# sandialabs/tenzing

Hardware: AMD Instinct MI355X
Metric: best-schedule iter time (ms) + MCTS search wall-clock, 3D halo-exchange 8 ranks (lower is better)
Workload: dtype fp64

## Files before the change

### tenzing_amd/csrc/bind/module.cpp

```cpp
#include <pybind11/functional.h>
#include <pybind11/pybind11.h>
#include <pybind11/stl.h>

#include "core/benchmark.hpp"
#include "core/health.hpp"
#include "core/solve.hpp"
#include "hip/comm_ops.hpp"
#include "hip/hip_runtime.hpp"
#include "hip/rccl_comm.hpp"
#include "hip/rocsparse_spmv.hpp"
#include "kernels/kernels.hpp"
#include "workloads/workloads.hpp"

#include <hip/hip_runtime_api.h>

#include <csignal>
#include <cstdlib>
#include <execinfo.h>
#include <sstream>
#include <unistd.h>
#include <vector>

namespace py = pybind11;
using namespace tz;
// ... 930 lines not shown
      .def_readwrite("hostsplit_fracs", &HaloArgs::hostsplit_fracs)
      .def_readwrite("hostsplit_chunks", &HaloArgs::hostsplit_chunks)
      .def_readwrite("wide_puts", &HaloArgs::wide_puts)
      .def_readwrite("wide_put_blocks", &HaloArgs::wide_put_blocks)
      .def_readwrite("ipc_grid", &HaloArgs::ipc_grid)
      .def_readwrite("copy_puts", &HaloArgs::copy_puts)
      .def_readwrite("copy_engines", &HaloArgs::copy_engines)
      .def_readwrite("move_pairs", &HaloArgs::move_pairs)
      .def_readwrite("grid_memory", &HaloArgs::grid_memory)
      .def_readwrite("node_tag", &HaloArgs::node_tag)
      .def_readwrite("device", &HaloArgs::device)
      .def("json", [](const HaloArgs &a) { return a.json().dump(); });
  py::class_<HaloExchange, std::shared_ptr<HaloExchange>>(m, "HaloExchange")
      .def(py::init([](const HaloArgs &a) { return std::make_shared<HaloExchange>(a); }))
      .def_property_readonly("args", &HaloExchange::args)
      .def("ndirs", &HaloExchange::ndirs)
      .def("dir_name", [](const HaloExchange &h, int i) { return h.dir(i).name(); })
      .def("dir", [](const HaloExchange &h, int i) { auto d = h.dir(i); return py::make_tuple(d.dx, d.dy, d.dz); })
      .def("opposite", &HaloExchange::opposite)
      .def("neighbor", &HaloExchange::neighbor)
      .def("coords", &HaloExchange::coords)
      .def("rank_grid", &HaloExchange::rank_grid)
      .def("box_elems", &HaloExchange::box_elems)
      .def("pack_box", [](const HaloExchange &h, int i) { return box_to_dict(h.pack_box(i)); })
      .def("unpack_box", [](const HaloExchange &h, int i) { return box_to_dict(h.unpack_box(i)); })
      .def_static("chunk_box",
                  [](const py::dict &b, int parts) {
                    py::list out;
                    for (const kern::BoxDesc &c : HaloExchange::chunk_box(box_from_dict(b), parts))
                      out.append(box_to_dict(c));
                    return out;
                  },
                  py::arg("box"), py::arg("parts"))
      .def("grid_elems", &HaloExchange::grid_elems)
      .def("grid_memory", &HaloExchange::grid_memory, "fine or coarse (HaloArgs.grid_memory)")
      .def("off_node_dirs", &HaloExchange::off_node_dirs,
           "remote directions whose neighbour runs on another node (RCCL only)")
      .def("layout", [](const HaloExchange &h) {
             const kern::HaloGeom g = h.geom();
             py::dict d;
             d["order"] = g.order == 0 ? "xyzq" : "qxyz";
             d["x_offset_cells"] = g.xoff;
             d["row_pitch_elems"] = g.sy;
             d["grid_bytes"] = double(h.grid_elems()) * 8.0;
             const bool q = g.order == 1;
             d["strides_qzyx"] = py::make_tuple(q ? 1 : g.sq, g.sz, g.sy, q ? int64_t(g.nq) : 1);
             d["shape_qzyx"] = py::make_tuple(g.nq, g.nz + 2 * g.g, g.ny + 2 * g.g, g.nx + 2 * g.g);
             d["ghost"] = g.g;
             return d;
           }, "storage layout: order, x padding before the first ghost cell, row pitch")
      .def("exchange_bytes", &HaloExchange::exchange_bytes)
      .def("setup", [](HaloExchange &h, Ctrl *c) { h.setup(c); }, py::arg("ctrl") = nullptr,
           py::call_guard<py::gil_scoped_release>())
      .def("ready", &HaloExchange::ready)
      .def("add_to_graph", &HaloExchange::add_to_graph)
      .def("grid_ptr", [](const HaloExchange &h) { return reinterpret_cast<uintptr_t>(h.grid()); })
      .def("read_grid", [](HaloExchange &h, uintptr_t dst, uintptr_t s) { h.copy_grid(P(dst), false, P(s)); },
           py::arg("dst"), py::arg("stream") = 0, "copy grid_elems() doubles of storage to dst")
      .def("write_grid", [](HaloExchange &h, uintptr_t src, uintptr_t s) { h.copy_grid(P(src), true, P(s)); },
           py::arg("src"), py::arg("stream") = 0, "overwrite the grid storage from src")
      .def("init_grid", [](HaloExchange &h, uintptr_t s, int gen) { h.init_grid(P(s), gen); },
           py::arg("stream") = 0, py::arg("gen") = 0)
      .def("check_grid", [](HaloExchange &h, uintptr_t s) { return h.check_grid(P(s)); }, py::arg("stream") = 0)
      .def("check_stencil", [](HaloExchange &h, uintptr_t s) { return h.check_stencil(P(s)); }, py::arg("stream") = 0)
      .def("stencil", [](const HaloExchange &h, int region, uintptr_t s) { h.stencil(region, P(s)); },
           py::arg("region"), py::arg("stream") = 0)
// ... 312 lines not shown
```

### tenzing_amd/csrc/workloads/halo.cpp

```cpp
#include "halo_internal.hpp"

#include <functional>
#include <map>

#include "core/health.hpp"
#include "core/solve.hpp"

#include <algorithm>
#include <chrono>
#include <thread>

namespace tz {

Json HaloArgs::json() const {
  Json j;
  j["nx"] = nx;
  j["ny"] = ny;
  j["nz"] = nz;
  j["nq"] = nq;
  j["ghost"] = ghost;
  j["neighbors"] = neighbors;
  j["order"] = order;
  j["transport"] = transport;
  j["fuse"] = fuse;
// ... 148 lines not shown
  copyEngines_ = a_.copy_engines;

  TZ_CHECK(a_.relay == "auto" || a_.relay == "off" || a_.relay == "force",
           "relay must be auto, off or force (got " << a_.relay << ")");
  TZ_CHECK(!a_.relay_fracs.empty(), "relay_fracs is empty");
  for (double f : a_.relay_fracs) TZ_CHECK(f > 0.0 && f < 0.5, "relay fraction " << f << " not in (0, 0.5)");
  bool facesIpc = true;
  for (int i : group_dirs(1)) facesIpc = facesIpc && ipc_[i];
  relay_ = a_.relay != "off" && a_.px == 2 && a_.py == 2 && a_.pz == 2 && useIpc_ && !ipcGrid_ && facesIpc;
  TZ_CHECK(a_.relay != "force" || relay_,
           "relay routing forced but needs a 2x2x2 rank grid with ipc puts in buffers mode");
  TZ_CHECK(a_.hostsplit == "auto" || a_.hostsplit == "off" || a_.hostsplit == "force",
           "hostsplit must be auto, off or force (got " << a_.hostsplit << ")");
  TZ_CHECK(!a_.hostsplit_fracs.empty(), "hostsplit_fracs is empty");
  for (double f : a_.hostsplit_fracs)
    TZ_CHECK(f > 0.0 && f < 1.0, "host share " << f << " not in (0, 1)");
  TZ_CHECK(a_.hostsplit_chunks >= 1 && a_.hostsplit_chunks <= 8,
           "hostsplit_chunks must be 1..8 (got " << a_.hostsplit_chunks << ")");
  hsChunks_ = a_.hostsplit_chunks;
  bool anyFace = false;
  for (int i : group_dirs(1)) anyFace = anyFace || ipc_[i];
  hsOffered_ = a_.hostsplit != "off" && useIpc_ && !ipcGrid_ && anyFace;
  TZ_CHECK(a_.hostsplit != "force" || hsOffered_,
           "host split forced but needs remote faces with ipc puts in buffers mode");
  corner_ = coord_to_rank(cx_ + 1, cy_ + 1, cz_ + 1);
  relayOrigin_ = coord_to_rank(cx_ - 1, cy_ - 1, cz_ - 1);
  fwdTo_.assign(dirs_.size(), -1);
  fwdFrom_.assign(dirs_.size(), -1);
  for (size_t i = 0; i < dirs_.size(); ++i) {
    const Dir &d = dirs_[i];
    fwdTo_[i] = coord_to_rank(cx_ - 1 + d.dx, cy_ - 1 + d.dy, cz_ - 1 + d.dz);
    fwdFrom_[i] = coord_to_rank(cx_ - d.dx + 1, cy_ - d.dy + 1, cz_ - d.dz + 1);
  }
}

HaloExchange::~HaloExchange() {
  if (recoveryHook_) remove_recovery_hook(recoveryHook_);
  for (auto &kv : engines_) {
    for (void *e : kv.second.events) (void)hipEventDestroy(static_cast<hipEvent_t>(e));
    for (void *s : kv.second.streams) (void)hipStreamDestroy(static_cast<hipStream_t>(s));
  }
  for (void *p : opened_) (void)hipIpcCloseMemHandle(p);
  if (flags_) (void)hipFree(flags_);
}

int HaloExchange::coord_to_rank(int x, int y, int z) const {
  auto w = [](int v, int n) { return ((v % n) + n) % n; };
  return w(x, a_.px) + a_.px * (w(y, a_.py) + a_.py * w(z, a_.pz));
}

static void axis_range(int d, int n, int g, bool ghost, int &lo, int &ext) {
  if (d == 0) {
    lo = g;
    ext = n;
  } else if (d < 0) {
    lo = ghost ? 0 : g;
    ext = g;
  } else {
    lo = ghost ? n + g : n;
    ext = g;
  }
}

kern::BoxDesc halo_detail::make_box(const HaloArgs &a, const HaloExchange::Dir &d, bool ghost,
                                    int64_t xoff, int64_t sy, int64_t sz, int64_t sq) {
  int x0, ex, y0, ey, z0, ez;
  axis_range(d.dx, a.nx, a.ghost, ghost, x0, ex);
  axis_range(d.dy, a.ny, a.ghost, ghost, y0, ey);
  axis_range(d.dz, a.nz, a.ghost, ghost, z0, ez);
  kern::BoxDesc b;
  if (a.order == "xyzq") {
    b.grid_off = z0 * sz + y0 * sy + x0 + xoff;
    b.len = ex;
    b.n1 = ey;
    b.n2 = ez;
    b.n3 = a.nq;
    b.s1 = sy;
    b.s2 = sz;
    b.s3 = sq;
  } else {
    b.grid_off = int64_t(a.nq) * (x0 + xoff) + y0 * sy + z0 * sz;
    b.len = a.nq * ex;
    b.n1 = ey;
    b.n2 = ez;
    b.n3 = 1;
    b.s1 = sy;
    b.s2 = sz;
    b.s3 = 0;
  }
  return b;
}

kern::BoxDesc HaloExchange::pack_box(int i) const {
  kern::BoxDesc b = make_box(a_, dirs_[i], false, xoff_, sy_, sz_, sq_);
  if (!send_.empty()) b.buf = send_[i].as<double>();
  return b;
}

kern::BoxDesc HaloExchange::unpack_box(int i) const {
  kern::BoxDesc b = make_box(a_, dirs_[i], true, xoff_, sy_, sz_, sq_);
  if (!recv_.empty()) b.buf = recv_[i].as<double>();
  ghost_widening(dirs_[i].dx, b.grid_off, b.len, b.lead, b.trail);
  return b;
}

size_t HaloExchange::box_elems(int i) const {
  kern::BoxDesc b = make_box(a_, dirs_[i], false, xoff_, sy_, sz_, sq_);
  return size_t(b.len) * b.n1 * b.n2 * b.n3;
}

double HaloExchange::exchange_bytes() const {
  double s = 0;
  for (int i = 0; i < ndirs(); ++i) s += 8.0 * double(box_elems(i));
  return s;
}

kern::HaloGeom HaloExchange::geom() const {
  kern::HaloGeom g;
  g.order = a_.order == "xyzq" ? 0 : 1;
  g.xoff = xoff_;
  g.sy = sy_;
  g.sz = sz_;
  g.sq = sq_;
  g.nx = a_.nx;
  g.ny = a_.ny;
  g.nz = a_.nz;
  g.nq = a_.nq;
  g.g = a_.ghost;
  g.cx = cx_;
  g.cy = cy_;
  g.cz = cz_;
  g.px = a_.px;
  g.py = a_.py;
  g.pz = a_.pz;
// ... 6 lines not shown
  if (ready()) return;
  ctrl_ = ctrl;
  if (a_.device >= 0) TZ_HIP(hipSetDevice(a_.device));
  TZ_CHECK(a_.grid_memory >= -1 && a_.grid_memory <= 1, "grid_memory must be -1 (auto), 0 or 1");
  if (useIpc_ && ctrl && ctrl->size() > 1) {
    const std::vector<std::string> ids = ctrl->allgather(node_identity() + a_.node_tag);
    TZ_CHECK(int(ids.size()) == a_.size, "allgather returned " << ids.size() << " entries");
    std::vector<double> off(size_t(ndirs()), 0.0);
    for (int i = 0; i < ndirs(); ++i)
      if (ipc_[i] && ids[size_t(nbr_[i])] != ids[size_t(a_.rank)]) off[size_t(i)] = 1.0;
    ctrl->allreduce_max(off.data(), int(off.size()));
    offNode_.assign(size_t(ndirs()), 0);
    int n = 0;
    for (int i = 0; i < ndirs(); ++i)
      if (off[size_t(i)] != 0.0) {
        offNode_[size_t(i)] = 1;
        ipc_[i] = false;
        ++n;
      }
    if (n > 0) {
      TZ_CHECK(a_.transport == "auto", "transport " << a_.transport << ": " << n
                   << " directions have a neighbour on another node, which IPC cannot reach "
                      "(transport auto sends them over RCCL)");
      useIpc_ = std::any_of(ipc_.begin(), ipc_.end(), [](bool b) { return b; });
      relay_ = false;
      hsOffered_ = false;
      useCopy_ = useIpc_ && a_.copy_puts;
      TZ_LOG(Info, "halo: " << n << " directions cross nodes (RCCL), "
                            << std::count(ipc_.begin(), ipc_.end(), true) << " stay on IPC");
    }
  }
  gridFine_ = a_.grid_memory < 0 ? useIpc_ && ipcGrid_ : a_.grid_memory != 0;
  grid_ = DeviceBuffer(gridElems_ * sizeof(double), gridFine_);
  send_.resize(ndirs());
  recv_.resize(ndirs());
  for (int i = 0; i < ndirs(); ++i) {
    if (direct_[i]) continue;
    if (pipe_[i] || (ipc_[i] && useCopy_ && !ipcGrid_)) send_[i] = DeviceBuffer(box_elems(i) * sizeof(double));
    if (pipe_[i] || (ipc_[i] && !ipcGrid_))
      recv_[i] = DeviceBuffer((box_elems(opp_[i]) + 16 * ((relay_ ? 1 : 0) + (hsOffered_ ? hsChunks_ + 1 : 0))) *
                                  sizeof(double),
                              ipc_[i] && !ipcGrid_);
  }
  if (relay_) {
    relayBuf_.resize(ndirs());
    for (int i : relay_faces()) {
      size_t most = 0;
      for (double f : a_.relay_fracs) {
        kern::BoxDesc A, B;
        split_box(make_box(a_, dirs_[i], false, xoff_, sy_, sz_, sq_), f, A, B);
        most = std::max(most, size_t(B.len) * B.n1 * B.n2 * B.n3);
      }
      relayBuf_[i] = DeviceBuffer(most * sizeof(double), true);
    }
  }
  const std::string failEnv = std::getenv("TZ_FAIL_TRANSPORTS") ? std::getenv("TZ_FAIL_TRANSPORTS") : "";
  auto simulated = [&](const std::string &what) {
    return ("," + failEnv + ",").find("," + what + ",") != std::string::npos;
  };
  if (useIpc_) {
    std::string why = setup_ipc(ctrl);
    if (why.empty() && simulated("ipc")) why = "simulated failure (TZ_FAIL_TRANSPORTS)";
    double failed = why.empty() ? 0.0 : 1.0;
    ctrl->allreduce_max(&failed, 1);
    ipcReady_ = failed == 0.0;
    if (!ipcReady_) {
      ipcWhy_ = why.empty() ? "failed on another rank" : why;
      TZ_LOG(Warn, "ipc transport unavailable: " << ipcWhy_);
      TZ_CHECK(a_.transport != "ipc", "ipc transport requested but unavailable: " << why);
    }
    if (relay_) {
      double bad = relayWhy_.empty() ? 0.0 : 1.0;
      ctrl->allreduce_max(&bad, 1);
      relayReady_ = ipcReady_ && bad == 0.0;
      if (ipcReady_ && !relayReady_) {
        TZ_LOG(Warn, "relay routing unavailable"
// ... 36 lines not shown
    ctrl->allreduce_max(&failed, 1);
    if (failed != 0.0) drop_rccl(why.empty() ? "communicator creation failed on another rank" : why);
  }
  init_grid();
  if (useRccl_) {
    const std::string why = rccl_preflight(*ctrl);
    if (!why.empty()) {
      drop_rccl("preflight: " + why);
    } else {
      if (!rcclGraphOk_) TZ_LOG(Warn, "RCCL ops run eagerly only: " << rcclGraphWhy_);
      TZ_LOG(Info, "rccl preflight passed (" << comms_.size() << " communicators of "
                                             << rccl_nranks() << " ranks)"
                                             << (rcclGraphOk_ ? ", " + rcclCaptureNote_ : ", eager only"));
    }
    init_grid();
  }
  if (useIpc_ && ipcReady_) {
    TZ_HIP(hipDeviceSynchronize());
    ctrl->barrier();
    ipc_preflight(ctrl);
    if (ipcReady_ && useCopy_ && !ipcGrid_) copy_preflight(ctrl);
    if (ipcReady_) wide_put_preflight(ctrl);
    if (relay_ && ipcReady_) relay_preflight(ctrl);
    if (hsReady_ && ipcReady_) hostsplit_preflight(ctrl);
  }
  bool piped = false;
  for (int i = 0; i < ndirs(); ++i) piped = piped || pipe_[i];
  if (piped && !useRccl_ && a_.transport != "copy" && !useHost_) {
    if (!off_node_dirs().empty() && useIpc_ && ipcReady_) {
      ipcReady_ = false;
      ipcWhy_ = "RCCL unavailable for the directions that cross nodes: host-staged transport";
    }
    if (useIpc_ && ipcReady_) {
      for (int i = 0; i < ndirs(); ++i) {
        if (pipe_[i]) {
          pipe_[i] = false;
          if (!(ipc_[i] && useCopy_ && !ipcGrid_)) send_[i] = DeviceBuffer();
          if (ipcGrid_) recv_[i] = DeviceBuffer();
        }
      }
    } else {
      TZ_CHECK(a_.transport == "auto", "RCCL transport unavailable and no fallback: " << rcclWhy_);
      useHost_ = true;
      TZ_LOG(Warn, "no device transport works (rccl: " << rcclWhy_ << "; ipc: "
                                                     << (useIpc_ ? ipcWhy_ : "not offered")
                                                     << "): the host-staged transport carries "
                                                        "the remote directions");
    }
  }
  TZ_HIP(hipDeviceSynchronize());
  if (useIpc_ && ipcReady_) {
    ctrl->barrier();
    recoveryHook_ = add_recovery_hook([this](Ctrl &c) { reset_ipc_counters(&c); });
  }
}

void HaloExchange::drop_rccl(const std::string &why) {
  for (auto &c : comms_)
    if (c && !c->aborted()) c->abort();
  comms_.clear();
  useRccl_ = false;
  rcclWhy_ = why;
  TZ_LOG(Warn, "RCCL transport unavailable: " << why);
}

int HaloExchange::rccl_nranks() const { return comms_.empty() ? 0 : comms_.front()->size(); }

std::map<std::string, std::string> HaloExchange::transport_report() const {
  std::map<std::string, std::string> r;
  const bool remote = std::any_of(nbr_.begin(), nbr_.end(), [&](int n) { return n != a_.rank; });
  const std::string &t = a_.transport;
  if (useRccl_)
    r["rccl"] = rcclGraphOk_ ? (rcclCaptureNote_.empty() ? "ok" : "ok (hipGraph: " + rcclCaptureNote_ + ")")
// ... 225 lines not shown
  TZ_HIP(hipStreamSynchronize(s));
}

void HaloExchange::check_pipelined(int i) const {
  TZ_CHECK(i >= 0 && i < ndirs(), "direction " << i << " out of range");
  TZ_CHECK(!direct_[i], "direction " << dirs_[i].name()
                                     << " uses the direct transport (no pack/transfer/unpack)");
  TZ_CHECK(pipe_[i] || ipc_[i], "direction " << dirs_[i].name() << " has no staging buffers");
  TZ_CHECK(ready(), "halo not set up");
}

void HaloExchange::pack(int i, void *stream) const {
  check_pipelined(i);
  kern::box_copy(grid(), pack_box(i), false, stream);
}

void HaloExchange::unpack(int i, void *stream) const {
  check_pipelined(i);
  kern::box_copy(grid(), unpack_box(i), true, stream);
}

const RcclComm &HaloExchange::comm_for(int streamIdx, int dir) const {
  TZ_CHECK(!comms_.empty(), "no RCCL communicators");
  const int k = streamIdx >= 0 ? streamIdx : dir;
  return *comms_[size_t(k) % comms_.size()];
}

void HaloExchange::shift(int i, void *stream, int streamIdx) const {
  check_pipelined(i);
  const int o = opp_[i];
  const size_t n = box_elems(i);
  if (useRccl_) {
    const RcclComm &c = comm_for(streamIdx, i);
    c.sendrecv(send_[i].get(), n, nbr_[i], recv_[o].get(), n, nbr_[o], 1, stream);
  } else {
    TZ_CHECK(nbr_[i] == a_.rank, "shift " << dirs_[i].name() << ": the neighbour is remote and RCCL "
                                          "is not in use (host transport: he_hostxfer)");
    kern::CopyDesc c{recv_[o].get(), send_[i].get(), n * sizeof(double)};
    kern::copy_many(&c, 1, stream);
  }
}

std::vector<int> HaloExchange::all_dirs() const {
  std::vector<int> v;
  for (int i = 0; i < ndirs(); ++i) v.push_back(i);
  return v;
}

std::vector<int> HaloExchange::group_dirs(int k) const {
  std::vector<int> v;
  for (int i = 0; i < ndirs(); ++i) {
    const int a = (dirs_[i].dx != 0) + (dirs_[i].dy != 0) + (dirs_[i].dz != 0);
    if (a == k || (k == 0 && a >= 2)) v.push_back(i);
  }
  return v;
}

void HaloExchange::pack_group(const std::vector<int> &dirs, void *stream) const {
  std::vector<kern::BoxDesc> bs;
  for (int i : dirs) {
    check_pipelined(i);
    bs.push_back(pack_box(i));
  }
  for (size_t k = 0; k < bs.size(); k += kern::kMaxBoxes)
    kern::box_copy_many(grid(), bs.data() + k, int(std::min<size_t>(kern::kMaxBoxes, bs.size() - k)),
                        false, stream);
}

void HaloExchange::unpack_group(const std::vector<int> &dirs, void *stream) const {
  std::vector<kern::BoxDesc> bs;
  for (int i : dirs) {
    check_pipelined(i);
    bs.push_back(unpack_box(opp_[i]));
  }
  for (size_t k = 0; k < bs.size(); k += kern::kMaxBoxes)
    kern::box_copy_many(grid(), bs.data() + k, int(std::min<size_t>(kern::kMaxBoxes, bs.size() - k)),
                        true, stream);
}

void HaloExchange::shift_group(const std::vector<int> &dirs, void *stream, int streamIdx) const {
  if (dirs.empty()) return;
  for (int i : dirs) check_pipelined(i);
  if (useRccl_) {
    std::vector<RcclComm::Xfer> xs;
    for (int i : dirs) {
      const int o = opp_[i];
      const size_t n = box_elems(i);
      xs.push_back({send_[i].get(), n, nbr_[i], recv_[o].get(), n, nbr_[o]});
    }
    comm_for(streamIdx, dirs.front()).exchange(xs, 1, stream);
  } else {
    std::vector<kern::CopyDesc> cs;
    for (int i : dirs) {
      TZ_CHECK(nbr_[i] == a_.rank, "shift " << dirs_[i].name() << ": the neighbour is remote and "
                                            "RCCL is not in use (host transport: he_hostxfer)");
      cs.push_back({recv_[opp_[i]].get(), send_[i].get(), box_elems(i) * sizeof(double)});
    }
    for (size_t k = 0; k < cs.size(); k += kern::kMaxBoxes)
      kern::copy_many(cs.data() + k, int(std::min<size_t>(kern::kMaxBoxes, cs.size() - k)), stream);
  }
}

std::vector<kern::MoveDesc> HaloExchange::direct_moves(const std::vector<int> &dirs_in) const {
  std::vector<int> dirs = dirs_in;
  std::stable_sort(dirs.begin(), dirs.end(), [&](int a, int b) {
    auto k = [&](int i) { return (dirs_[i].dx != 0) + (dirs_[i].dy != 0) + (dirs_[i].dz != 0); };
    return k(a) < k(b);
  });
  std::vector<kern::MoveDesc> ms;
  for (int i : dirs) {
    TZ_CHECK(i >= 0 && i < ndirs() && direct_[i], "direction " << i << " is not a direct (self) transfer");
    const kern::BoxDesc s = make_box(a_, dirs_[i], false, xoff_, sy_, sz_, sq_);
    const kern::BoxDesc d = make_box(a_, dirs_[opp_[i]], true, xoff_, sy_, sz_, sq_);
    kern::MoveDesc m;
    m.src = grid();
    m.dst = grid();
    m.src_off = s.grid_off;
    m.dst_off = d.grid_off;
    m.s1 = s.s1;
    m.s2 = s.s2;
    m.s3 = s.s3;
    m.len = s.len;
    m.n1 = s.n1;
    m.n2 = s.n2;
    m.n3 = s.n3;
    if (a_.ghost_align > 0) widen_to_sectors(dirs_[opp_[i]].dx, m);
    ms.push_back(m);
  }
  if (a_.order == "xyzq" && a_.move_pairs) ms = pair_x_moves(ms);
// ... 144 lines not shown
  } else {
    const int64_t end = dstOff % rowLen + len;
    const int64_t e = (A - (dstOff + len) % A) % A;
    if (end + e <= rowLen) trail = int32_t(e);
  }
}

void HaloExchange::widen_to_sectors(int ghostDx, kern::MoveDesc &m) const {
  int32_t lead = 0, trail = 0;
  ghost_widening(ghostDx, m.dst_off, m.len, lead, trail);
  m.src_off -= lead;
  m.dst_off -= lead;
  m.len += lead + trail;
}

std::vector<int> HaloExchange::pipelined_dirs() const {
  std::vector<int> v;
  for (int i = 0; i < ndirs(); ++i)
    if (!direct_[i]) v.push_back(i);
  return v;
}

void HaloExchange::host_exchange(const std::vector<int> &dirs_in) const {
  TZ_CHECK(ready() && ctrl_, "halo not set up");
  std::vector<int> dirs = dirs_in;
  std::sort(dirs.begin(), dirs.end());
  std::vector<std::string> out(size_t(a_.size));
  for (int i : dirs) {
    check_pipelined(i);
    const size_t bytes = box_elems(i) * sizeof(double);
    std::string &o = out[size_t(nbr_[i])];
    const size_t at = o.size();
    o.resize(at + bytes);
    TZ_HIP(hipMemcpy(&o[at], send_[i].get(), bytes, hipMemcpyDeviceToHost));
  }
  const std::vector<std::string> in = ctrl_->alltoallv(out);
  std::vector<size_t> used(in.size(), 0);
  for (int i : dirs) {
    const int o = opp_[i];
    const size_t from = size_t(nbr_[o]);
    const size_t bytes = box_elems(i) * sizeof(double);
    TZ_CHECK(from < in.size() && used[from] + bytes <= in[from].size(),
             "host exchange: rank " << from << " sent " << in[from].size() << " bytes, fewer than expected");
    TZ_HIP(hipMemcpy(recv_[o].get(), in[from].data() + used[from], bytes, hipMemcpyHostToDevice));
    used[from] += bytes;
  }
  for (size_t r = 0; r < in.size(); ++r)
    TZ_CHECK(used[r] == in[r].size(), "host exchange: rank " << r << " sent " << in[r].size()
                                                              << " bytes, expected " << used[r]);
}

void HaloExchange::pack_all(void *stream) const { pack_group(pipelined_dirs(), stream); }
void HaloExchange::unpack_all(void *stream) const { unpack_group(pipelined_dirs(), stream); }
void HaloExchange::shift_all(void *stream) const { shift_group(pipelined_dirs(), stream); }

}
```

### tenzing_amd/csrc/workloads/halo_ipc.cpp

```cpp
#include "halo_internal.hpp"

namespace tz {

void HaloExchange::off_node_exchange(void *stream) const {
  const std::vector<int> far = off_node_dirs();
  if (far.empty()) return;
  TZ_CHECK(useRccl_, "directions that cross nodes need the RCCL transport");
  for (int i : far) pack(i, stream);
  for (int i : far) shift(i, stream);
  for (int i : far) unpack(opp_[i], stream);
}

void HaloExchange::ipc_preflight(Ctrl *ctrl) {
  std::vector<int> local, remote;
  for (int i = 0; i < ndirs(); ++i) {
    if (direct_[i]) local.push_back(i);
    else if (ipc_[i]) remote.push_back(i);
  }
  double bad = 0;
  std::string why;
  const double keep = ipcTimeoutS_;
  ipcTimeoutS_ = std::min(ipcTimeoutS_, preflight_wait_s());
  for (int gen = 1; gen <= 2 && bad == 0; ++gen) {
    if (gen > 1) {
// ... 174 lines not shown
  init_grid();
}

std::string HaloExchange::setup_ipc(Ctrl *ctrl) {
  TZ_CHECK(ctrl && ctrl->size() == a_.size, "ipc transport needs a control plane of size " << a_.size);
  if (const char *v = std::getenv("TZ_IPC_TIMEOUT")) ipcTimeoutS_ = std::atof(v);
  const size_t nd = size_t(ndirs());
  const size_t H = sizeof(hipIpcMemHandle_t);
  std::string mine, err;
  try {
    TZ_HIP(hipExtMallocWithFlags(&flags_, kSlotSets * nd * 8, hipDeviceMallocUncached));
    TZ_HIP(hipMemset(flags_, 0, kSlotSets * nd * 8));
    expected_ = DeviceBuffer(nd * 8);
    TZ_HIP(hipMemset(expected_.get(), 0, nd * 8));
    sent_ = DeviceBuffer(nd * 8);
    TZ_HIP(hipMemset(sent_.get(), 0, nd * 8));
    relayBook_ = DeviceBuffer(4 * nd * 8);
    TZ_HIP(hipMemset(relayBook_.get(), 0, relayBook_.bytes()));
    done_ = DeviceBuffer(4 * nd * kern::kMaxBoxes * sizeof(unsigned int));
    TZ_HIP(hipMemset(done_.get(), 0, done_.bytes()));
    err_ = DeviceBuffer(sizeof(int));
    TZ_HIP(hipMemset(err_.get(), 0, sizeof(int)));
    TZ_HIP(hipDeviceSynchronize());
    auto handle_of = [&](void *p) {
      hipIpcMemHandle_t h;
      std::memset(&h, 0, sizeof(h));
      if (p) TZ_HIP(hipIpcGetMemHandle(&h, p));
      return std::string(reinterpret_cast<const char *>(&h), H);
    };
    mine = node_identity() + handle_of(flags_);
    if (ipcGrid_) {
      mine += handle_of(grid());
    } else {
      for (int i = 0; i < ndirs(); ++i) mine += handle_of(ipc_[i] ? recv_[i].get() : nullptr);
      if (relay_)
        for (int i = 0; i < ndirs(); ++i)
          mine += handle_of(size_t(i) < relayBuf_.size() ? relayBuf_[i].get() : nullptr);
    }
    TZ_LOG(Info, "ipc: exported " << (ipcGrid_ ? "grid" : "receive buffers") << " and flags");
  } catch (const std::exception &e) {
    err = std::string("export: ") + e.what();
    mine.clear();
  }
  const std::vector<std::string> all = ctrl->allgather(mine);
  if (!err.empty()) return err;
  const std::string me = node_identity();
  auto open = [&](const std::string &blob, size_t k) {
    TZ_CHECK(blob.size() >= kNodeIdBytes + (k + 1) * H, "a peer exported no IPC handles");
    TZ_CHECK(blob.compare(0, kNodeIdBytes, me) == 0, "a peer runs on another node");
    const char *at = blob.data() + kNodeIdBytes + k * H;
    hipIpcMemHandle_t h;
    std::memcpy(&h, at, H);
    TZ_CHECK(std::any_of(at, at + H, [](char c) { return c != 0; }),
             "a peer exported no IPC handle in slot " << k);
    void *p = nullptr;
    TZ_HIP(hipIpcOpenMemHandle(&p, h, hipIpcMemLazyEnablePeerAccess));
    opened_.push_back(p);
    return p;
  };
  try {
    TZ_CHECK(int(all.size()) == a_.size, "allgather returned " << all.size() << " entries");
    peerGrid_.assign(size_t(a_.size), nullptr);
    peerFlags_.assign(size_t(a_.size), nullptr);
    peerRecv_.assign(nd, nullptr);
    for (int i = 0; i < ndirs(); ++i) {
      if (!ipc_[i]) continue;
      const int q = nbr_[i];
      const std::string &blob = all[size_t(q)];
      if (!peerFlags_[size_t(q)]) {
        TZ_LOG(Info, "ipc: mapping rank " << q);
        peerFlags_[size_t(q)] = open(blob, 0);
        if (ipcGrid_) peerGrid_[size_t(q)] = open(blob, 1);
      }
      if (!ipcGrid_) peerRecv_[size_t(i)] = open(blob, 1 + size_t(opp_[i]));
    }
  } catch (const std::exception &e) {
    return std::string("map: ") + e.what();
  }
  if (relay_) {
    relayWhy_.clear();
    try {
      auto flags_of = [&](int q) {
        if (!peerFlags_[size_t(q)]) {
          TZ_LOG(Info, "ipc: mapping rank " << q << " (relay)");
          peerFlags_[size_t(q)] = open(all[size_t(q)], 0);
        }
      };
      peerRelay_.assign(nd, nullptr);
      peerFwdRecv_.assign(nd, nullptr);
      flags_of(corner_);
      flags_of(relayOrigin_);
      for (int i : relay_faces()) {
        flags_of(fwdTo_[i]);
        flags_of(fwdFrom_[i]);
        peerRelay_[size_t(i)] = open(all[size_t(corner_)], 1 + nd + size_t(i));
        peerFwdRecv_[size_t(i)] = open(all[size_t(fwdTo_[i])], 1 + size_t(opp_[i]));
      }
    } catch (const std::exception &e) {
      relayWhy_ = std::string("relay map: ") + e.what();
    }
  }
  return "";
}

std::map<int, int> HaloExchange::ipc_peer_devices() const {
  std::map<int, int> out;
  for (size_t q = 0; q < peerFlags_.size(); ++q) {
    if (!peerFlags_[q]) continue;
    hipPointerAttribute_t at{};
    out[int(q)] = hipPointerGetAttributes(&at, peerFlags_[q]) == hipSuccess ? at.device : -1;
  }
  return out;
}

void HaloExchange::put_group(const std::vector<int> &dirs, void *stream, int max_blocks) const {
  TZ_CHECK(ready() && ipcReady_, "ipc transport not set up");
  TZ_CHECK(!dirs.empty() && dirs.size() <= size_t(kern::kMaxBoxes), "bad put group");
  std::vector<kern::MoveDesc> ms;
  std::vector<kern::BoxDesc> bs;
  kern::MoveSignal sig;
  sig.max_blocks = max_blocks;
  sig.done = done_.as<unsigned int>() + size_t(dirs.front()) * kern::kMaxBoxes;
  kern::ipc_wait(static_cast<const unsigned long long *>(flags_) + ndirs(), sent_.as<unsigned long long>(),
                 dirs.data(), int(dirs.size()), err_.as<int>(), ipcTimeoutS_, stream, 1);
  for (size_t k = 0; k < dirs.size(); ++k) {
    const int i = dirs[k];
    TZ_CHECK(i >= 0 && i < ndirs() && ipc_[i], "direction " << i << " is not an ipc put");
    const int q = nbr_[i];
    sig.flag[k] = static_cast<unsigned long long *>(peerFlags_[size_t(q)]) + i;
    if (!ipcGrid_) {
      kern::BoxDesc b = make_box(a_, dirs_[i], false, xoff_, sy_, sz_, sq_);
      b.buf = static_cast<double *>(peerRecv_[size_t(i)]);
      bs.push_back(b);
      continue;
    }
    const kern::BoxDesc s = make_box(a_, dirs_[i], false, xoff_, sy_, sz_, sq_);
    const kern::BoxDesc d = make_box(a_, dirs_[opp_[i]], true, xoff_, sy_, sz_, sq_);
    kern::MoveDesc m;
    m.src = grid();
    m.dst = static_cast<double *>(peerGrid_[size_t(q)]);
    m.src_off = s.grid_off;
    m.dst_off = d.grid_off;
    m.s1 = s.s1;
    m.s2 = s.s2;
    m.s3 = s.s3;
    m.len = s.len;
    m.n1 = s.n1;
    m.n2 = s.n2;
    m.n3 = s.n3;
    ms.push_back(m);
  }
  if (ipcGrid_) kern::box_move_many_signal(ms.data(), int(ms.size()), sig, stream);
  else kern::box_pack_many_signal(grid(), bs.data(), int(bs.size()), sig, stream);
}

void HaloExchange::copy_put_group(const std::vector<int> &dirs, void *stream, bool sdma) const {
  TZ_CHECK(ready() && ipcReady_ && useCopy_ && !ipcGrid_, "ipc copy-engine puts not set up");
  TZ_CHECK(!dirs.empty() && dirs.size() <= size_t(kern::kMaxBoxes), "bad copy-put group");
  hipStream_t s = static_cast<hipStream_t>(stream);
  std::vector<kern::BoxDesc> bs;
  std::vector<unsigned long long *> arrive;
  for (int i : dirs) {
    TZ_CHECK(i >= 0 && i < ndirs() && ipc_[i] && send_[i].get() && peerRecv_[size_t(i)],
             "direction " << i << " is not a copy-engine put");
    bs.push_back(pack_box(i));
    arrive.push_back(static_cast<unsigned long long *>(peerFlags_[size_t(nbr_[i])]) + i);
  }
  kern::ipc_wait(static_cast<const unsigned long long *>(flags_) + ndirs(), sent_.as<unsigned long long>(),
                 dirs.data(), int(dirs.size()), err_.as<int>(), ipcTimeoutS_, stream, 1);
  kern::box_copy_many(grid(), bs.data(), int(bs.size()), false, stream);
  std::vector<Copy> cs;
  for (int i : dirs) cs.push_back({peerRecv_[size_t(i)], send_[i].get(), box_elems(i) * sizeof(double)});
  engine_copies(cs, s, sdma);
  kern::ipc_signal(arrive.data(), int(arrive.size()), stream);
}

HaloExchange::EngineSet &HaloExchange::engines_for(void *stream) const {
  std::lock_guard<std::mutex> lk(enginesMu_);
  EngineSet &e = engines_[stream];
  if (e.events.empty()) {
    hipStreamCaptureMode mode = hipStreamCaptureModeRelaxed;
    TZ_HIP(hipThreadExchangeStreamCaptureMode(&mode));
    try {
      for (int k = 1; k < copyEngines_; ++k) {
        hipStream_t st = nullptr;
        TZ_HIP(hipStreamCreateWithFlags(&st, hipStreamNonBlocking));
        e.streams.push_back(st);
      }
      for (int k = 0; k < copyEngines_; ++k) {
        hipEvent_t ev = nullptr;
        TZ_HIP(hipEventCreateWithFlags(&ev, hipEventDisableTiming));
        e.events.push_back(ev);
      }
    } catch (...) {
      (void)hipThreadExchangeStreamCaptureMode(&mode);
      throw;
    }
    TZ_HIP(hipThreadExchangeStreamCaptureMode(&mode));
  }
  return e;
}

void HaloExchange::engine_copies(const std::vector<Copy> &copies, void *stream, bool sdma) const {
  hipStream_t s = static_cast<hipStream_t>(stream);
  const hipMemcpyKind kind = sdma ? hipMemcpyDeviceToDeviceNoCU : hipMemcpyDeviceToDevice;
// ... 214 lines not shown
```

### tenzing_amd/csrc/workloads/workloads.hpp

```cpp
#pragma once

#include "core/ctrl.hpp"
#include "core/graph.hpp"
#include "kernels/kernels.hpp"

#include <array>
#include <map>
#include <memory>
#include <mutex>
#include <string>
#include <vector>

namespace tz {

class RcclComm;
class RocsparseCsr;

double preflight_limit_s(double dflt);

class DeviceBuffer {
public:
  DeviceBuffer() = default;
  explicit DeviceBuffer(size_t bytes);
  DeviceBuffer(size_t bytes, bool peerWritten);
// ... 125 lines not shown
  std::string hostsplit = "auto";
  std::vector<double> hostsplit_fracs = {0.1, 0.2, 0.3, 0.4};
  int hostsplit_chunks = 1;
  std::string wide_puts = "auto";
  int wide_put_blocks = 256;
  int device = -1;
  Json json() const;
};

class HaloExchange : public std::enable_shared_from_this<HaloExchange> {
public:
  struct Dir {
    int dx, dy, dz;
    std::string name() const;
  };

  explicit HaloExchange(HaloArgs a);
  ~HaloExchange();

  const HaloArgs &args() const { return a_; }
  int ndirs() const { return int(dirs_.size()); }
  const Dir &dir(int i) const { return dirs_[i]; }
  int opposite(int i) const { return opp_[i]; }
  int neighbor(int i) const { return nbr_[i]; }
  std::array<int, 3> coords() const { return {cx_, cy_, cz_}; }
  std::array<int, 3> rank_grid() const { return {a_.px, a_.py, a_.pz}; }
  int coord_to_rank(int x, int y, int z) const;
  kern::BoxDesc pack_box(int i) const;
  kern::BoxDesc unpack_box(int i) const;
  size_t box_elems(int i) const;
  size_t grid_elems() const { return gridElems_; }
  double exchange_bytes() const;
  kern::HaloGeom geom() const;

  void setup(Ctrl *ctrl);
  bool ready() const { return grid_.get() != nullptr; }
  void add_to_graph(Graph &g);
  void add_exchange(Graph &g);

  double *grid() const { return grid_.as<double>(); }
  void init_grid(void *stream = nullptr, int gen = 0);
  uint64_t check_grid(void *stream = nullptr);
  void copy_grid(void *ptr, bool toGrid, void *stream = nullptr);
  uint64_t check_stencil(void *stream = nullptr);
  void stencil(int region, void *stream) const;
  double *stencil_out() const { return out_.as<double>(); }

  void pack(int i, void *stream) const;
  void unpack(int i, void *stream) const;
  void shift(int i, void *stream, int streamIdx = -1) const;
  void pack_all(void *stream) const;
  void unpack_all(void *stream) const;
  void shift_all(void *stream) const;
  void pack_group(const std::vector<int> &dirs, void *stream) const;
  void unpack_group(const std::vector<int> &dirs, void *stream) const;
  void shift_group(const std::vector<int> &dirs, void *stream, int streamIdx = -1) const;
  std::vector<int> all_dirs() const;
  std::vector<int> pipelined_dirs() const;
  std::vector<int> group_dirs(int k) const;
  bool uses_rccl() const { return useRccl_; }
  bool rccl_graph_ok() const { return rcclGraphOk_; }
  bool uses_direct() const { return useDirect_; }
  bool uses_ipc() const { return useIpc_; }
  bool uses_host() const { return useHost_; }
  int rccl_nranks() const;
  std::map<std::string, std::string> transport_report() const;
// ... 116 lines not shown
  EngineSet &engines_for(void *stream) const;
  struct Copy {
    void *dst;
    const void *src;
    size_t bytes;
  };
  void engine_copies(const std::vector<Copy> &copies, void *stream, bool sdma = true) const;
  void *flags_ = nullptr;
  static constexpr int kSlotSets = 6;
  DeviceBuffer expected_, done_, err_;
  DeviceBuffer sent_;
  DeviceBuffer relayBook_;
  bool relay_ = false, relayReady_ = false;
  std::string relayWhy_;
  int corner_ = -1;
  std::vector<DeviceBuffer> relayBuf_;
  std::vector<void *> peerRelay_;
  std::vector<void *> peerFwdRecv_;
  std::vector<int> fwdTo_, fwdFrom_;
  int relayOrigin_ = -1;
  void split_box(const kern::BoxDesc &b, double frac, kern::BoxDesc &A, kern::BoxDesc &B) const;
  void relay_preflight(Ctrl *ctrl);
  unsigned long long *peer_slot(int rank, int set, int i) const;
  std::vector<unsigned long long *> credit_ptrs(const std::vector<int> &dirs) const;
  const RcclComm &comm_for(int streamIdx, int dir) const;
  std::vector<kern::MoveDesc> pair_x_moves(const std::vector<kern::MoveDesc> &ms) const;
  void widen_to_sectors(int ghostDx, kern::MoveDesc &m) const;
  void ghost_widening(int ghostDx, int64_t dstOff, int32_t len, int32_t &lead, int32_t &trail) const;
  static constexpr int kDefaultComms = 4;
  bool ipcGrid_ = true;
  bool gridFine_ = false;
  std::vector<char> offNode_;
  std::vector<void *> peerGrid_, peerFlags_;
  std::vector<void *> peerRecv_;
  std::vector<void *> opened_;
  double ipcTimeoutS_ = 10.0;
  DeviceBuffer grid_;
  std::vector<DeviceBuffer> send_, recv_;
  std::vector<std::shared_ptr<RcclComm>> comms_;
  DeviceBuffer count_;
  DeviceBuffer out_;
  kern::StencilBox stencil_box(int x0, int x1, int y0, int y1, int z0, int z1) const;
};


struct CsrHost {
  int64_t rows = 0, cols = 0;
  std::vector<int32_t> rowPtr, colInd;
  std::vector<float> val;
  int64_t nnz() const { return int64_t(colInd.size()); }
};

CsrHost random_band_matrix(int64_t n, int64_t bw, int64_t nnz, uint64_t seed);
CsrHost read_matrix_market(const std::string &path);
void write_matrix_market(const CsrHost &A, const std::string &path);
std::pair<int64_t, int64_t> row_partition(int64_t n, int rank, int size);

struct SpmvArgs {
  std::string matrix = "";
  int64_t m = 150000;
  int64_t bw = 0;
  int64_t nnz = 0;
  int64_t nnz_actual = 0;
  uint64_t seed = 1;
  int rank = 0, size = 1;
  int device = -1;
  bool compound = true;
  bool kernel_choice = true;
  std::string library = "adaptive";
  std::string form = "choice";
  std::string transport = "auto";
// ... 82 lines not shown
```

Baseline: 0.04436.

## Pack halo send/recv buffers into per-peer contiguous arenas and coalesce transfers

Replaces the per-direction send and receive device buffers with one send arena and one receive arena. Slices for directions going to the same neighbour rank sit next to each other, with matching offsets on the sender and receiver sides. The RCCL exchange and the copy-engine IPC puts now merge adjacent slices into one transfer per run, so fewer, larger messages and copies are issued. IPC now exports and maps one handle per rank instead of one per direction. The merged transfers also carry the 256-byte alignment padding and slack between slices, which adds some bytes to each message.

New measurement: 0.04440. No clear change (+0.1%).

```diff
diff --git a/tenzing_amd/csrc/bind/module.cpp b/tenzing_amd/csrc/bind/module.cpp
--- a/tenzing_amd/csrc/bind/module.cpp
+++ b/tenzing_amd/csrc/bind/module.cpp
@@ -986,6 +986,17 @@
                     return out;
                   },
                   py::arg("box"), py::arg("parts"))
+      .def("send_spans", [](const HaloExchange &h) {
+             py::list out;
+             for (const auto &s : h.send_spans()) out.append(py::make_tuple(s.peer, s.offset, s.bytes));
+             return out;
+           }, "per direction (peer, byte offset, bytes) of its slice of the send arena (offset -1: "
+              "a direct self move, no slice); no setup needed")
+      .def("recv_spans", [](const HaloExchange &h) {
+             py::list out;
+             for (const auto &s : h.recv_spans()) out.append(py::make_tuple(s.peer, s.offset, s.bytes));
+             return out;
+           }, "per ghost side (peer, byte offset, bytes) of its slice of the receive arena")
       .def("grid_elems", &HaloExchange::grid_elems)
       .def("grid_memory", &HaloExchange::grid_memory, "fine or coarse (HaloArgs.grid_memory)")
       .def("off_node_dirs", &HaloExchange::off_node_dirs,
diff --git a/tenzing_amd/csrc/workloads/halo.cpp b/tenzing_amd/csrc/workloads/halo.cpp
--- a/tenzing_amd/csrc/workloads/halo.cpp
+++ b/tenzing_amd/csrc/workloads/halo.cpp
@@ -204,6 +204,61 @@
     fwdTo_[i] = coord_to_rank(cx_ - 1 + d.dx, cy_ - 1 + d.dy, cz_ - 1 + d.dz);
     fwdFrom_[i] = coord_to_rank(cx_ - d.dx + 1, cy_ - d.dy + 1, cz_ - d.dz + 1);
   }
+  layout_arenas();
+}
+
+void HaloExchange::layout_arenas() {
+  const size_t nd = dirs_.size();
+  sliceSlack_ = 16 * ((relay_ ? 1 : 0) + (hsOffered_ ? hsChunks_ + 1 : 0));
+  sendOff_.assign(nd, -1);
+  recvOff_.assign(nd, -1);
+  std::vector<char> placed(nd, 0);
+  int64_t at = 0;
+  for (size_t i = 0; i < nd; ++i) {
+    if (direct_[i] || placed[i]) continue;
+    for (size_t j = i; j < nd; ++j) {
+      if (direct_[j] || placed[j] || nbr_[j] != nbr_[i]) continue;
+      placed[j] = 1;
+      sendOff_[j] = at;
+      recvOff_[size_t(opp_[j])] = at;
+      at += round_up(slice_bytes(int(j)), 256);
+    }
+  }
+  arenaBytes_ = at;
+}
+
+std::vector<HaloExchange::Span> HaloExchange::send_spans() const {
+  std::vector<Span> v;
+  for (int i = 0; i < ndirs(); ++i)
+    v.push_back({nbr_[i], sendOff_[size_t(i)], sendOff_[size_t(i)] < 0 ? 0 : slice_bytes(i)});
+  return v;
+}
+
+std::vector<HaloExchange::Span> HaloExchange::recv_spans() const {
+  std::vector<Span> v;
+  for (int i = 0; i < ndirs(); ++i)
+    v.push_back({nbr_[i], recvOff_[size_t(i)], recvOff_[size_t(i)] < 0 ? 0 : slice_bytes(opp_[i])});
+  return v;
+}
+
+std::vector<HaloExchange::Run> HaloExchange::send_runs(const std::vector<int> &dirs_in) const {
+  std::vector<int> dirs = dirs_in;
+  std::sort(dirs.begin(), dirs.end(), [&](int a, int b) { return sendOff_[size_t(a)] < sendOff_[size_t(b)]; });
+  std::vector<Run> runs;
+  int last = -1;
+  for (int i : dirs) {
+    TZ_CHECK(i >= 0 && i < ndirs() && sendOff_[size_t(i)] >= 0, "direction " << i << " has no staging slice");
+    const int64_t off = sendOff_[size_t(i)], payload = int64_t(box_elems(i)) * 8;
+    if (last >= 0 && nbr_[last] == nbr_[i] &&
+        sendOff_[size_t(last)] + round_up(slice_bytes(last), 256) == off) {
+      runs.back().bytes = off + payload - runs.back().offset;
+    } else {
+      TZ_CHECK(last < 0 || off > sendOff_[size_t(last)], "direction " << i << " listed twice");
+      runs.push_back({i, off, payload});
+    }
+    last = i;
+  }
+  return runs;
 }
 
 HaloExchange::~HaloExchange() {
@@ -265,13 +320,13 @@
 
 kern::BoxDesc HaloExchange::pack_box(int i) const {
   kern::BoxDesc b = make_box(a_, dirs_[i], false, xoff_, sy_, sz_, sq_);
-  if (!send_.empty()) b.buf = send_[i].as<double>();
+  b.buf = static_cast<double *>(send_buf(i));
   return b;
 }
 
 kern::BoxDesc HaloExchange::unpack_box(int i) const {
   kern::BoxDesc b = make_box(a_, dirs_[i], true, xoff_, sy_, sz_, sq_);
-  if (!recv_.empty()) b.buf = recv_[i].as<double>();
+  b.buf = static_cast<double *>(recv_buf(i));
   ghost_widening(dirs_[i].dx, b.grid_off, b.len, b.lead, b.trail);
   return b;
 }
@@ -344,16 +399,15 @@
   }
   gridFine_ = a_.grid_memory < 0 ? useIpc_ && ipcGrid_ : a_.grid_memory != 0;
   grid_ = DeviceBuffer(gridElems_ * sizeof(double), gridFine_);
-  send_.resize(ndirs());
-  recv_.resize(ndirs());
+  bool needSend = false, needRecv = false, peerWritten = false;
   for (int i = 0; i < ndirs(); ++i) {
     if (direct_[i]) continue;
-    if (pipe_[i] || (ipc_[i] && useCopy_ && !ipcGrid_)) send_[i] = DeviceBuffer(box_elems(i) * sizeof(double));
-    if (pipe_[i] || (ipc_[i] && !ipcGrid_))
-      recv_[i] = DeviceBuffer((box_elems(opp_[i]) + 16 * ((relay_ ? 1 : 0) + (hsOffered_ ? hsChunks_ + 1 : 0))) *
-                                  sizeof(double),
-                              ipc_[i] && !ipcGrid_);
-  }
+    needSend = needSend || pipe_[i] || (ipc_[i] && useCopy_ && !ipcGrid_);
+    needRecv = needRecv || pipe_[i] || (ipc_[i] && !ipcGrid_);
+    peerWritten = peerWritten || (ipc_[i] && !ipcGrid_);
+  }
+  if (needSend) sendArena_ = DeviceBuffer(size_t(arenaBytes_));
+  if (needRecv) recvArena_ = DeviceBuffer(size_t(arenaBytes_), peerWritten);
   if (relay_) {
     relayBuf_.resize(ndirs());
     for (int i : relay_faces()) {
@@ -456,13 +510,13 @@
       ipcWhy_ = "RCCL unavailable for the directions that cross nodes: host-staged transport";
     }
     if (useIpc_ && ipcReady_) {
+      bool copyPuts = false;
       for (int i = 0; i < ndirs(); ++i) {
-        if (pipe_[i]) {
-          pipe_[i] = false;
-          if (!(ipc_[i] && useCopy_ && !ipcGrid_)) send_[i] = DeviceBuffer();
-          if (ipcGrid_) recv_[i] = DeviceBuffer();
-        }
+        pipe_[i] = false;
+        copyPuts = copyPuts || (ipc_[i] && useCopy_ && !ipcGrid_);
       }
+      if (!copyPuts) sendArena_ = DeviceBuffer();
+      if (ipcGrid_) recvArena_ = DeviceBuffer();
     } else {
       TZ_CHECK(a_.transport == "auto", "RCCL transport unavailable and no fallback: " << rcclWhy_);
       useHost_ = true;
@@ -754,11 +808,11 @@
   const size_t n = box_elems(i);
   if (useRccl_) {
     const RcclComm &c = comm_for(streamIdx, i);
-    c.sendrecv(send_[i].get(), n, nbr_[i], recv_[o].get(), n, nbr_[o], 1, stream);
+    c.sendrecv(send_buf(i), n, nbr_[i], recv_buf(o), n, nbr_[o], 1, stream);
   } else {
     TZ_CHECK(nbr_[i] == a_.rank, "shift " << dirs_[i].name() << ": the neighbour is remote and RCCL "
                                           "is not in use (host transport: he_hostxfer)");
-    kern::CopyDesc c{recv_[o].get(), send_[i].get(), n * sizeof(double)};
+    kern::CopyDesc c{recv_buf(o), send_buf(i), n * sizeof(double)};
     kern::copy_many(&c, 1, stream);
   }
 }
@@ -805,10 +859,10 @@
   for (int i : dirs) check_pipelined(i);
   if (useRccl_) {
     std::vector<RcclComm::Xfer> xs;
-    for (int i : dirs) {
-      const int o = opp_[i];
-      const size_t n = box_elems(i);
-      xs.push_back({send_[i].get(), n, nbr_[i], recv_[o].get(), n, nbr_[o]});
+    for (const Run &r : send_runs(dirs)) {
+      const size_t n = size_t(r.bytes) / sizeof(double);
+      xs.push_back({sendArena_.as<char>() + r.offset, n, nbr_[r.first],
+                    recvArena_.as<char>() + r.offset, n, nbr_[opp_[r.first]]});
     }
     comm_for(streamIdx, dirs.front()).exchange(xs, 1, stream);
   } else {
@@ -816,7 +870,7 @@
     for (int i : dirs) {
       TZ_CHECK(nbr_[i] == a_.rank, "shift " << dirs_[i].name() << ": the neighbour is remote and "
                                             "RCCL is not in use (host transport: he_hostxfer)");
-      cs.push_back({recv_[opp_[i]].get(), send_[i].get(), box_elems(i) * sizeof(double)});
+      cs.push_back({recv_buf(opp_[i]), send_buf(i), box_elems(i) * sizeof(double)});
     }
     for (size_t k = 0; k < cs.size(); k += kern::kMaxBoxes)
       kern::copy_many(cs.data() + k, int(std::min<size_t>(kern::kMaxBoxes, cs.size() - k)), stream);
@@ -1027,7 +1081,7 @@
     std::string &o = out[size_t(nbr_[i])];
     const size_t at = o.size();
     o.resize(at + bytes);
-    TZ_HIP(hipMemcpy(&o[at], send_[i].get(), bytes, hipMemcpyDeviceToHost));
+    TZ_HIP(hipMemcpy(&o[at], send_buf(i), bytes, hipMemcpyDeviceToHost));
   }
   const std::vector<std::string> in = ctrl_->alltoallv(out);
   std::vector<size_t> used(in.size(), 0);
@@ -1037,7 +1091,7 @@
     const size_t bytes = box_elems(i) * sizeof(double);
     TZ_CHECK(from < in.size() && used[from] + bytes <= in[from].size(),
              "host exchange: rank " << from << " sent " << in[from].size() << " bytes, fewer than expected");
-    TZ_HIP(hipMemcpy(recv_[o].get(), in[from].data() + used[from], bytes, hipMemcpyHostToDevice));
+    TZ_HIP(hipMemcpy(recv_buf(o), in[from].data() + used[from], bytes, hipMemcpyHostToDevice));
     used[from] += bytes;
   }
   for (size_t r = 0; r < in.size(); ++r)
diff --git a/tenzing_amd/csrc/workloads/halo_ipc.cpp b/tenzing_amd/csrc/workloads/halo_ipc.cpp
--- a/tenzing_amd/csrc/workloads/halo_ipc.cpp
+++ b/tenzing_amd/csrc/workloads/halo_ipc.cpp
@@ -230,12 +230,12 @@
     if (ipcGrid_) {
       mine += handle_of(grid());
     } else {
-      for (int i = 0; i < ndirs(); ++i) mine += handle_of(ipc_[i] ? recv_[i].get() : nullptr);
+      mine += handle_of(recvArena_.get());
       if (relay_)
         for (int i = 0; i < ndirs(); ++i)
           mine += handle_of(size_t(i) < relayBuf_.size() ? relayBuf_[i].get() : nullptr);
     }
-    TZ_LOG(Info, "ipc: exported " << (ipcGrid_ ? "grid" : "receive buffers") << " and flags");
+    TZ_LOG(Info, "ipc: exported " << (ipcGrid_ ? "grid" : "receive arena") << " and flags");
   } catch (const std::exception &e) {
     err = std::string("export: ") + e.what();
     mine.clear();
@@ -260,6 +260,7 @@
     TZ_CHECK(int(all.size()) == a_.size, "allgather returned " << all.size() << " entries");
     peerGrid_.assign(size_t(a_.size), nullptr);
     peerFlags_.assign(size_t(a_.size), nullptr);
+    peerArena_.assign(size_t(a_.size), nullptr);
     peerRecv_.assign(nd, nullptr);
     for (int i = 0; i < ndirs(); ++i) {
       if (!ipc_[i]) continue;
@@ -269,8 +270,10 @@
         TZ_LOG(Info, "ipc: mapping rank " << q);
         peerFlags_[size_t(q)] = open(blob, 0);
         if (ipcGrid_) peerGrid_[size_t(q)] = open(blob, 1);
-      }
-      if (!ipcGrid_) peerRecv_[size_t(i)] = open(blob, 1 + size_t(opp_[i]));
+        else peerArena_[size_t(q)] = open(blob, 1);
+      }
+      if (!ipcGrid_)
+        peerRecv_[size_t(i)] = static_cast<char *>(peerArena_[size_t(q)]) + recvOff_[size_t(opp_[i])];
     }
   } catch (const std::exception &e) {
     return std::string("map: ") + e.what();
@@ -284,6 +287,10 @@
           peerFlags_[size_t(q)] = open(all[size_t(q)], 0);
         }
       };
+      auto arena_of = [&](int q) {
+        if (!peerArena_[size_t(q)]) peerArena_[size_t(q)] = open(all[size_t(q)], 1);
+        return static_cast<char *>(peerArena_[size_t(q)]);
+      };
       peerRelay_.assign(nd, nullptr);
       peerFwdRecv_.assign(nd, nullptr);
       flags_of(corner_);
@@ -291,8 +298,8 @@
       for (int i : relay_faces()) {
         flags_of(fwdTo_[i]);
         flags_of(fwdFrom_[i]);
-        peerRelay_[size_t(i)] = open(all[size_t(corner_)], 1 + nd + size_t(i));
-        peerFwdRecv_[size_t(i)] = open(all[size_t(fwdTo_[i])], 1 + size_t(opp_[i]));
+        peerRelay_[size_t(i)] = open(all[size_t(corner_)], 2 + size_t(i));
+        peerFwdRecv_[size_t(i)] = arena_of(fwdTo_[i]) + recvOff_[size_t(opp_[i])];
       }
     } catch (const std::exception &e) {
       relayWhy_ = std::string("relay map: ") + e.what();
@@ -359,7 +366,7 @@
   std::vector<kern::BoxDesc> bs;
   std::vector<unsigned long long *> arrive;
   for (int i : dirs) {
-    TZ_CHECK(i >= 0 && i < ndirs() && ipc_[i] && send_[i].get() && peerRecv_[size_t(i)],
+    TZ_CHECK(i >= 0 && i < ndirs() && ipc_[i] && send_buf(i) && peerRecv_[size_t(i)],
              "direction " << i << " is not a copy-engine put");
     bs.push_back(pack_box(i));
     arrive.push_back(static_cast<unsigned long long *>(peerFlags_[size_t(nbr_[i])]) + i);
@@ -368,7 +375,8 @@
                  dirs.data(), int(dirs.size()), err_.as<int>(), ipcTimeoutS_, stream, 1);
   kern::box_copy_many(grid(), bs.data(), int(bs.size()), false, stream);
   std::vector<Copy> cs;
-  for (int i : dirs) cs.push_back({peerRecv_[size_t(i)], send_[i].get(), box_elems(i) * sizeof(double)});
+  for (const Run &r : send_runs(dirs))
+    cs.push_back({peerRecv_[size_t(r.first)], send_buf(r.first), size_t(r.bytes)});
   engine_copies(cs, s, sdma);
   kern::ipc_signal(arrive.data(), int(arrive.size()), stream);
 }
diff --git a/tenzing_amd/csrc/workloads/workloads.hpp b/tenzing_amd/csrc/workloads/workloads.hpp
--- a/tenzing_amd/csrc/workloads/workloads.hpp
+++ b/tenzing_amd/csrc/workloads/workloads.hpp
@@ -181,6 +181,13 @@
   size_t grid_elems() const { return gridElems_; }
   double exchange_bytes() const;
   kern::HaloGeom geom() const;
+  struct Span {
+    int peer;
+    int64_t offset;
+    int64_t bytes;
+  };
+  std::vector<Span> send_spans() const;
+  std::vector<Span> recv_spans() const;
 
   void setup(Ctrl *ctrl);
   bool ready() const { return grid_.get() != nullptr; }
@@ -363,11 +370,28 @@
   bool gridFine_ = false;
   std::vector<char> offNode_;
   std::vector<void *> peerGrid_, peerFlags_;
+  std::vector<void *> peerArena_;
   std::vector<void *> peerRecv_;
   std::vector<void *> opened_;
   double ipcTimeoutS_ = 10.0;
   DeviceBuffer grid_;
-  std::vector<DeviceBuffer> send_, recv_;
+  DeviceBuffer sendArena_, recvArena_;
+  std::vector<int64_t> sendOff_, recvOff_;
+  int64_t sliceSlack_ = 0;
+  int64_t arenaBytes_ = 0;
+  int64_t slice_bytes(int i) const { return int64_t(box_elems(i) + size_t(sliceSlack_)) * 8; }
+  void *send_buf(int i) const {
+    return sendArena_.get() && sendOff_[size_t(i)] >= 0 ? sendArena_.as<char>() + sendOff_[size_t(i)] : nullptr;
+  }
+  void *recv_buf(int i) const {
+    return recvArena_.get() && recvOff_[size_t(i)] >= 0 ? recvArena_.as<char>() + recvOff_[size_t(i)] : nullptr;
+  }
+  struct Run {
+    int first;
+    int64_t offset, bytes;
+  };
+  std::vector<Run> send_runs(const std::vector<int> &dirs) const;
+  void layout_arenas();
   std::vector<std::shared_ptr<RcclComm>> comms_;
   DeviceBuffer count_;
   DeviceBuffer out_;
```
